# doughtmw/hmd-ego-pose

Hardware: AMD Instinct MI355X
Metric: frames/sec at 256x256 bs16 EfficientPose-phi0; ADD(-S) vs ref (higher is better)
Workload: dtype bf16; 1 GPU; EfficientPose phi=0 256x256 bf16 batch=16 per GPU: forward (stem, MBConv, BiFPN, 5 heads) + box/translation decode; seeded random-init weights, N(0,1) frames resident in HBM; 4 batches of 16 in flight per GPU on 4 HIP streams; phi=0, size=256, batch_per_gpu=16, global_batch=16, parallelism=dp1, batches_in_flight=4, anchors=12276, submission_threads=4

## Files before the change

### hmd_ego_pose_amd/csrc/hep_api.cpp

```cpp
#include <stdio.h>
#include <stdlib.h>
#include <string.h>

#include <math.h>

#include <chrono>
#include <fstream>
#include <memory>

#include "hep.h"
#include "hep_api_util.h"
#include "hep_plan.h"

using namespace hep;

thread_local std::string hep::g_err;

struct hep_handle { Session s; };

namespace hep {

Session::~Session() {
  if (!realised) return;
  for (auto& g : graphs) for (hipGraphExec_t ge : g.second) hipGraphExecDestroy(ge);
// ... 1070 lines not shown
  return calibrate_fp8(s, frames_nchw_device, batch);
} HEP_CATCH_INT

static std::string kernel_symbol(const Session& s, const Op& o) {
  const char* t = s.dtype ? "true" : "false";
  const int prec = o.kind == OP_PW ? (o.pw.fp8 ? 2 : (s.dtype ? 1 : 0)) : 0;
  char tmp[128];
  switch (o.kind) {
    case OP_STEM: if (o.stem.mfma) snprintf(tmp, sizeof tmp, "stem_kernel<%s, %d>", t, (o.stem.Cout + 15) / 16);
                  else snprintf(tmp, sizeof tmp, "stem_valu_kernel<%s>", t);
                  break;
    case OP_PW: { const int sev = pw_se_variant(o.pw);
                  const bool w8 = o.pw.nwv == 8 && prec == 0 && o.pw.mode == 2 && o.pw.act != ACT_SWISH && (sev == 0 || sev == 3) && o.pw.NT <= 2;
                  const bool fr = o.pw.frag && prec != 2 && o.pw.MT == 2 && o.pw.NT <= PW_FRAG_MAX_NT && o.pw.mode == 2 && sev >= 1 && o.pw.act != ACT_SWISH;
                  snprintf(tmp, sizeof tmp, fr ? "pw_gemm_kernel<%d, %d, %d, %d, %d, %d, %d, true>" : "pw_gemm_kernel<%d, %d, %d, %d, %d, %d, %d>", prec, o.pw.MT, o.pw.NT, o.pw.mode, o.pw.act == ACT_SWISH ? 1 : 0, sev, (w8 || (fr && o.pw.nwv == 8 && prec == 0 && sev == 3 && o.pw.NT <= 2)) ? 8 : 4); break; }
    case OP_DW: snprintf(tmp, sizeof tmp, "dw_kernel<%s, %d, %d, %d>", t, o.dw.k, o.dw.s, o.dw.TW); break;
    case OP_POOL: snprintf(tmp, sizeof tmp, "pool_kernel<%s>", t); break;
    case OP_PWG: snprintf(tmp, sizeof tmp, "pw_group_kernel<%s>", t); break;
    case OP_CHAIN: if (const int id = chain_shape_id(o.chain)) snprintf(tmp, sizeof tmp, "chain_shape_kernel<true, %d>", id);
                   else snprintf(tmp, sizeof tmp, "chain_kernel<%s, %d>", o.chain.bf16 ? "true" : "false", o.chain.stream_w);
                   break;
    case OP_SE: snprintf(tmp, sizeof tmp, "se_finish_kernel<%s>", t); break;
    case OP_MBF: { const int mp = o.mbf.has_expand && o.mbf.npass > 1 ? (o.mbf.mp_resident ? 2 : 1) : 0;
                   if (const int id = mbf_shape_id(o.mbf)) snprintf(tmp, sizeof tmp, "mbf_shape_kernel<%s, %d, %d, %d, %d, %d>", t, o.mbf.k, o.mbf.s, o.mbf.ts, mp, id);
                   else snprintf(tmp, sizeof tmp, "mbf_kernel<%s, %d, %d, %d, %s, %d>", t, o.mbf.k, o.mbf.s, o.mbf.ts, o.mbf.fp8 ? "true" : "false", mp);
                   break; }
#ifdef HEP_ALT
    case OP_SBF: snprintf(tmp, sizeof tmp, "sbf_kernel<%s>", t); break;
    case OP_LATE: snprintf(tmp, sizeof tmp, "late_kernel"); break;
    case OP_HEADS: snprintf(tmp, sizeof tmp, "heads_kernel"); break;
#endif
    case OP_XBF: { const int sp = xbf_specialised(o.xbf);
                   if (const int id = xbf_shape_id(o.xbf)) snprintf(tmp, sizeof tmp, "xbf_kernel_shape<true, %d>", id);
                   else snprintf(tmp, sizeof tmp, "xbf_kernel<%s, %d, %d, %d, %d, %d, %d, %d>", t, o.xbf.k, o.xbf.s, o.xbf.toh, o.xbf.tow, o.xbf.NT1, sp ? o.xbf.K1 : 0, sp ? o.xbf.NT2 : 0); break; }
    default: if (o.sep.direct) snprintf(tmp, sizeof tmp, "%s<%s, %d, %s>", o.sep.coop ? "tower_coop_kernel" : "tower_kernel", t, o.sep.C, o.sep.direct == 2 ? "true" : "false");
             else {
               const int mode = o.sep.chain ? 2 : (o.sep.nseg == 1 ? 0 : 1);
               const bool wl = o.sep.bf16 && o.sep.off_wpw && mode != 1;
               if (const int id = mode == 0 ? sep_shape_id(o.sep) : 0) snprintf(tmp, sizeof tmp, "sep_shape_kernel<true, %d>", id);
               else if (mode == 0 && sep_w8(o.sep)) snprintf(tmp, sizeof tmp, "sep_kernel<%s, 0, false, true>", t);
               else snprintf(tmp, sizeof tmp, wl ? "sep_kernel<%s, %d, true, false>" : "sep_kernel<%s, %d, false, false>", t, mode);
             }
             break;
  }
  return tmp;
}

// ... 124 lines not shown
```

### hmd_ego_pose_amd/csrc/hep_internal.h

```cpp
#pragma once
#include <hip/hip_runtime.h>
#include <stdint.h>

struct hep_sync;
struct GDSyncFailed { int rc; };

static constexpr inline uint32_t rcp_u32(uint32_t d) { return d <= 1 ? 0u : (uint32_t)(0x100000000ull / d) + 1u; }

#define HEP_MAX_SRC 3
#define SEP_MAX_TILES_N 6
#define SEP_MAX_TILES_MAP 24

enum { ACT_NONE = 0, ACT_SWISH = 1, ACT_SIGMOID = 2 };
enum { SRC_SAME = 1, SRC_UP = 2, SRC_DOWN = 3 };

struct StemArgs {
  const float* in; int64_t sn, sc, sh, sw;
  const float* w;
  const float* bias;
  void* out;
  int B, H, W, Ho, Wo, Cout, pad_t, pad_l, bf16;
  int mpw; uint32_t tx_rcp, ho_rcp;
  int mfma;
};
// ... 529 lines not shown
int backbone_tensor_count(const BGPlan&);
void backbone_tensor_offsets(const BGPlan&, int64_t* offsets);
int backbone_stage_count(const BGPlan&);
int backbone_stage(const BGPlan&, int i, char name[32], int64_t dims[4], int64_t* offset_floats);
void launch_backbone_forward(const BGPlan&, const float* params, const float* image, const float* branch_scale, float* const taps[3], float* ws, hipStream_t,
                             float momentum = 0.0f, float* stats_out = nullptr, const hep_sync* sync = nullptr);
void launch_backbone_backward(const BGPlan&, const float* const grad_taps[3], const float* branch_scale, float* grad_params, float* grad_image, float* ws,
                              hipStream_t, const hep_sync* sync = nullptr);

void launch_stem(const StemArgs&, hipStream_t);
int stem_uses_mfma(int cout, int force = -1);
void launch_pw(const PwArgs&, hipStream_t);
int pw_se_variant(const PwArgs&);
void launch_pwg(const PwgArgs&, hipStream_t);
void launch_dw(const DwArgs&, hipStream_t);
void launch_pool(const PoolArgs&, hipStream_t);
void launch_mbf(const MbfArgs&, hipStream_t);
size_t mbf_lds_layout(int Cin, int CC, int k, int s, int bf16, int has_expand, int max_inside, int ts, MbfArgs* a, int kp = 0);
int mbf_mp_fits(int CC, int kp, int bf16, int max_inside, int ts);
int mbf_mp_resident(int Cin, int CC, int max_inside, int ts);
int mbf_max_inside(int H, int W, int k, int s, int pad_t, int pad_l, int ts);
int mbf_prepare(void);
int mbf_shape_id(const MbfArgs&);
void launch_sep(const SepArgs&, hipStream_t);
void launch_tower(const SepArgs&, hipStream_t);
#define TOWER_BIAS_MAX 384
#define TOWER_WLDS_MAX (56 * 1024)
constexpr int tower_hdr_tiles(int C, bool bf16, int cap = 6) {
  if (!bf16) return 12;
  const long es = bf16 ? 2 : 4, wp = C + (bf16 ? 8 : 4), kstep = bf16 ? 32 : 16, ks = (C + kstep - 1) / kstep;
  const long fixed = 9L * C * 4 + 4L * ks * 64 * 16;
  const long room = TOWER_WLDS_MAX < 158L * 1024 - fixed ? TOWER_WLDS_MAX : 158L * 1024 - fixed;
  const long t = room / (16 * wp * es + 64);
  return t < 1 ? 1 : (t > cap ? cap : (int)t);
}
constexpr int tower_coop_hdr_tiles(int C, bool bf16) { return bf16 && C == 64 ? 36 : tower_hdr_tiles(C, bf16, 12); }
int tower_prepare(void);
int tower_coop_supported(int C, int bf16);
int tower_supports(int C);
int tower_map_tiles(int C);
void launch_decode(const DecodeArgs&, hipStream_t);
void launch_export(const ExportArgs&, hipStream_t);
void launch_preprocess(const PreprocArgs&, hipStream_t);
void launch_filter(const FilterArgs&, hipStream_t);
int filter_prepare(void);
void launch_amax_bf16(const void* x, int64_t n, unsigned* out , hipStream_t);
// ... 6 lines not shown
```

### hmd_ego_pose_amd/csrc/hep_plan.cpp

```cpp
#include <stdio.h>
#include <string.h>

#include <algorithm>
#include <cmath>
#include <map>

#include "hep.h"
#include "hep_plan.h"

namespace hep {

static const float kFusionEps = 1e-4f;

static void mbf_hpart_slot(Op& o, int seg, int idx, void* p) { SLOT(mbf.hpart)(o, seg, idx, p); SLOT(mbf.tail.hpart)(o, seg, idx, p); }

struct Planner {
  Session* s; const Pack& pk; std::string* err; WBuilder wb; bool ok = true;
  std::vector<Ref>& refs;
  int& ntails;
  const Knobs kn;
  std::map<int, int> front_of_out, front_of_part;
  Planner(Session* s_, const Pack& p, Plan* plan, std::string* e) : s(s_), pk(p), err(e), refs(plan->refs), ntails(plan->ntails), kn(s_->knobs) { wb.dtype = s_->dtype; wb.layout_only = plan->layout_only; }

  int tensor(const std::string& name, int H, int W, int C, bool f32 = false) {
// ... 343 lines not shown
      if (!boundary) flush_project();
      if (!ok) return -1;
    }
    auto dw_op = [&](OpKind kind, const std::string& name) {
      snprintf(nm, sizeof nm, "b%d.se_hpart", i);
      part_t = tensor(nm, 1, nblk, sqp, true);
      return new_op(kind, name);
    };
    auto dw_refs = [&](int op, Slot w, Slot bias, Slot se_wr, Slot in, Slot out, Slot part) {
      wref(op, w, wb.put_f32(wdw)); wref(op, bias, wb.put_f32(bn1.shift)); wref(op, se_wr, wr_off);
      if (in) tref(op, in, x, false);
      tref(op, out, dw_t, true); tref(op, part, part_t, true);
      Op& o = s->ops[op];
      o.act_bytes_per_image = ((double)Hin * Win + (double)Ho * Wo) * b.cexp * es();
      o.weight_bytes = (double)b.k * b.k * b.cexp * 4;
      o.flops_per_image = 2.0 * b.k * b.k * Ho * Wo * b.cexp;
    };
    auto mbf_op = [&](const char* suffix, int cin, int cc, int ts_, int has_expand, int max_in_, int npass_, int kp_) {
      nblk = ((Ho + ts_ - 1) / ts_) * ((Wo + ts_ - 1) / ts_) * ((b.cexp + cc - 1) / cc);
      const int op = dw_op(OP_MBF, "b" + std::to_string(i) + suffix);
      MbfArgs& m = s->ops[op].mbf;
      m.H = Hin; m.W = Win; m.Cin = cin; m.Cexp = b.cexp; m.Ho = Ho; m.Wo = Wo; m.k = b.k; m.s = b.stride;
      m.pad_t = pt; m.pad_l = pl; m.has_expand = has_expand; m.bf16 = s->dtype; m.CC = cc; m.sq = b.se; m.sqp = sqp; m.ts = ts_;
      m.npass = npass_; m.kp = kp_; m.generic = kn.mbf_generic != 0;
      mbf_lds_layout(cin, cc, b.k, b.stride, s->dtype, has_expand, max_in_, ts_, &m, kp_);
      front_of_out[dw_t] = op; front_of_part[part_t] = op;
      return op;
    };
    if (boundary) {
    } else if (CC) {
      if (!b.expand) CC = std::min(CC, b.cexp);
      const int op = mbf_op(".front", b.cin, CC, ts, b.expand, max_in, npass, kp);
      MbfArgs& m = s->ops[op].mbf;
      m.mp_resident = npass > 1 && mbf_mp_resident(b.cin, CC, max_in, ts) && kn.mbf_mp_res != 0;
      if (b.expand) {
        const PackTensor* w = get(p + "._expand_conv.conv.weight", {b.cexp, b.cin, 1, 1});
        BnFold bn0; if (!fold_bn(pk, p + "._bn0", b.cexp, &bn0, err)) ok = false;
        if (!ok) return -1;
        const int rows = (b.cexp + 15) / 16 * 16;
        const FoldedPw f = fold_pw(w, b.cin, nullptr, &bn0, 0, b.cexp, rows);
        if (s->dtype == 2) {
          std::vector<float> sc;
          wref(op, SLOT(mbf.we), wb.put_fp8(f.w, rows, b.cin, (b.cin + 15) & ~15, &sc)); wref(op, SLOT(mbf.we_scale), wb.put_f32(sc));
          m.fp8 = 1; m.a_scale = 1.f;
        } else wref(op, SLOT(mbf.we), wb.put_typed(f.w));
        wref(op, SLOT(mbf.be), wb.put_f32(bn0.shift));
      }
// ... 811 lines not shown
```

### hmd_ego_pose_amd/csrc/k_mbf.hip

```cpp
#include <stddef.h>
#include <stdio.h>
#include <stdlib.h>

#include <algorithm>

#include <type_traits>

#include "k_mbf_impl.h"

int mbf_shape_prepare_16(void); int mbf_shape_prepare_8(void);
bool launch_mbf_shape_16(int id, const MbfArgs&, dim3 grid, hipStream_t);
bool launch_mbf_shape_8(int id, const MbfArgs&, dim3 grid, hipStream_t);
void mbf_trace_bind_16(unsigned long long*); void mbf_trace_bind_8(unsigned long long*);

#ifdef HEP_MBF_TRACE
extern "C" int hep_dbg_mbf_trace(unsigned long long* host, int max_waves, int enable) {
  static unsigned long long* buf = nullptr;
  const size_t cap = (size_t)1 << 21;
  if (!buf) { if (hipMalloc((void**)&buf, cap * 8) != hipSuccess) return -1; hipMemset(buf, 0, cap * 8); }
  unsigned long long* p = enable ? buf : nullptr;
  mbf_trace_bind_tu(p); mbf_trace_bind_16(p); mbf_trace_bind_8(p);
  if (host) { hipDeviceSynchronize(); hipMemcpy(host, buf, (size_t)max_waves * 64, hipMemcpyDeviceToHost); }
  return (int)(cap / 8);
}
// ... 44 lines not shown
int mbf_mp_resident(int Cin, int CC, int max_inside, int ts) {
  const long items = (long)(((CC + 15) / 16) * 16 + max_inside) * (Cin / 8);
  return Cin % 8 == 0 && items <= 6L * mbf_threads(ts);
}

template <bool BF16, int KS, int S, int TS>
static int prep_one() {
  int rc = hipFuncSetAttribute(reinterpret_cast<const void*>(mbf_kernel<BF16, KS, S, TS, false, 0>), hipFuncAttributeMaxDynamicSharedMemorySize, 159 * 1024) == hipSuccess ? 0 : -1;
  rc |= hipFuncSetAttribute(reinterpret_cast<const void*>(mbf_kernel<BF16, KS, S, TS, false, 1>), hipFuncAttributeMaxDynamicSharedMemorySize, 159 * 1024) == hipSuccess ? 0 : -1;
  rc |= hipFuncSetAttribute(reinterpret_cast<const void*>(mbf_kernel<BF16, KS, S, TS, false, 2>), hipFuncAttributeMaxDynamicSharedMemorySize, 159 * 1024) == hipSuccess ? 0 : -1;
#ifdef HEP_WITH_FP8
  if constexpr (BF16) rc |= hipFuncSetAttribute(reinterpret_cast<const void*>(mbf_kernel<true, KS, S, TS, true, 0>), hipFuncAttributeMaxDynamicSharedMemorySize, 159 * 1024) == hipSuccess ? 0 : -1;
#endif
  return rc;
}
int mbf_prepare(void) {
  return prep_one<true, 3, 1, 8>() | prep_one<true, 3, 2, 8>() | prep_one<true, 5, 1, 8>() | prep_one<true, 5, 2, 8>() |
         prep_one<false, 3, 1, 8>() | prep_one<false, 3, 2, 8>() | prep_one<false, 5, 1, 8>() | prep_one<false, 5, 2, 8>() |
         prep_one<true, 3, 1, 16>() | prep_one<true, 5, 1, 16>() | prep_one<false, 3, 1, 16>() | prep_one<false, 5, 1, 16>() |
         mbf_shape_prepare_16() | mbf_shape_prepare_8();
}

int mbf_shape_id(const MbfArgs& a) {
  if (a.generic || a.fp8 || a.se_tail) return 0;
  const int mp = a.has_expand && a.npass > 1 ? (a.mp_resident ? 2 : 1) : 0;
#define X(id, bf, ks, s_, ts_, mp_, cin, cexp, cc, h, w, ho, wo, pt, pl, sq_, sqp_, he, of) \
  if ((a.bf16 != 0) == bf && a.k == ks && a.s == s_ && a.ts == ts_ && mp == mp_ && a.Cin == cin && a.Cexp == cexp && a.CC == cc && a.H == h && a.W == w && \
      a.Ho == ho && a.Wo == wo && a.pad_t == pt && a.pad_l == pl && a.sq == sq_ && a.sqp == sqp_ && (a.has_expand != 0) == (he != 0) && (a.out_frag != 0) == (of != 0)) return id;
  MBF_SHAPES(X)
#undef X
  return 0;
}

template <bool BF16, bool F8, int MP>
static void launch_mbf_t(const MbfArgs& a, dim3 grid, hipStream_t s) {
  if (a.ts == 16) {
    if (a.k == 3) hipLaunchKernelGGL((mbf_kernel<BF16, 3, 1, 16, F8, MP>), grid, dim3(1024), a.lds_bytes, s, a);
    else hipLaunchKernelGGL((mbf_kernel<BF16, 5, 1, 16, F8, MP>), grid, dim3(1024), a.lds_bytes, s, a);
  }
  else if (a.k == 3 && a.s == 1) hipLaunchKernelGGL((mbf_kernel<BF16, 3, 1, 8, F8, MP>), grid, dim3(512), a.lds_bytes, s, a);
  else if (a.k == 3 && a.s == 2) hipLaunchKernelGGL((mbf_kernel<BF16, 3, 2, 8, F8, MP>), grid, dim3(512), a.lds_bytes, s, a);
  else if (a.k == 5 && a.s == 1) hipLaunchKernelGGL((mbf_kernel<BF16, 5, 1, 8, F8, MP>), grid, dim3(512), a.lds_bytes, s, a);
  else hipLaunchKernelGGL((mbf_kernel<BF16, 5, 2, 8, F8, MP>), grid, dim3(512), a.lds_bytes, s, a);
}
void launch_mbf(const MbfArgs& a_, hipStream_t s) {
  MbfArgs a = a_;
#ifdef HEP_MBF_TRACE
  {
    static const char* sel = getenv("HEP_MBF_TRACE_SEL");
    int c = 0, h = 0;
    if (sel) sscanf(sel, "%d,%d", &c, &h);
    a.trace = !sel || (a.Cexp == c && a.H == h);
  }
#endif
  const int tiles = ((a.Wo + a.ts - 1) / a.ts) * ((a.Ho + a.ts - 1) / a.ts), chunks = (a.Cexp + a.CC - 1) / a.CC;
  dim3 grid(tiles * chunks, a.B);
  a.chunks = chunks; a.tiles_x = (a.Wo + a.ts - 1) / a.ts;
  a.chunks_rcp = rcp_u32(chunks); a.tiles_x_rcp = rcp_u32(a.tiles_x); a.gx_rcp = rcp_u32(grid.x);
#ifdef HEP_WITH_FP8
  if (a.bf16 && a.fp8) { launch_mbf_t<true, true, 0>(a, grid, s); return; }
#endif
  const int mp = a.has_expand && a.npass > 1 ? (a.mp_resident ? 2 : 1) : 0;
  a.vk_rcp = rcp_u32((uint32_t)std::max(1, a.Cin >> 3)); a.kpv_rcp = rcp_u32((uint32_t)std::max(1, a.kp >> 3));
  if (const int id = mbf_shape_id(a)) {
    if (launch_mbf_shape_16(id, a, grid, s) || launch_mbf_shape_8(id, a, grid, s)) return;
  }
  if (a.bf16) { if (mp == 2) launch_mbf_t<true, false, 2>(a, grid, s); else if (mp == 1) launch_mbf_t<true, false, 1>(a, grid, s); else launch_mbf_t<true, false, 0>(a, grid, s); }
  else { if (mp == 2) launch_mbf_t<false, false, 2>(a, grid, s); else if (mp == 1) launch_mbf_t<false, false, 1>(a, grid, s); else launch_mbf_t<false, false, 0>(a, grid, s); }
}
```

### hmd_ego_pose_amd/csrc/k_mbf_impl.h

```cpp
#pragma once
#include "hep_dev.h"
#include "hep_internal.h"
#include "se_finish.h"

#define MBF_SHAPES_16(X) \
  X(1, true, 5, 1, 16, 0,   40,  240, 64, 32, 32, 32, 32, 2, 2, 10, 16, 1, 0) \
  X(3, true, 3, 1, 16, 0,   80,  480, 64, 16, 16, 16, 16, 1, 1, 20, 24, 1, 1) \
  X(4, true, 5, 1, 16, 0,   80,  480, 64, 16, 16, 16, 16, 2, 2, 20, 24, 1, 1) \
  X(5, true, 5, 1, 16, 0,  112,  672, 64, 16, 16, 16, 16, 2, 2, 28, 32, 1, 1)
#define MBF_SHAPES_8(X) \
  X(2, true, 3, 2,  8, 0,   40,  240, 64, 32, 32, 16, 16, 0, 0, 10, 16, 1, 1) \
  X(6, true, 5, 2,  8, 0,  112,  672, 64, 16, 16,  8,  8, 1, 1, 28, 32, 1, 1) \
  X(7, true, 5, 1,  8, 0,  192, 1152, 64,  8,  8,  8,  8, 2, 2, 48, 48, 1, 1) \
  X(8, true, 3, 1,  8, 0,  192, 1152, 64,  8,  8,  8,  8, 1, 1, 48, 48, 1, 1)
#define MBF_SHAPES(X) MBF_SHAPES_16(X) MBF_SHAPES_8(X)

struct MbfShape { int Cin, Cexp, CC, H, W, Ho, Wo, pad_t, pad_l, sq, sqp, has_expand, out_frag; };
constexpr MbfShape mbf_shape(int d) {
  switch (d) {
#define X(id, bf, ks, s, ts, mp, cin, cexp, cc, h, w, ho, wo, pt, pl, sq, sqp, he, of) case id: return MbfShape{cin, cexp, cc, h, w, ho, wo, pt, pl, sq, sqp, he, of};
    MBF_SHAPES(X)
#undef X
    default: return MbfShape{};
  }
}


#ifdef HEP_MBF_TRACE
static __device__ unsigned long long* g_mbf_trace = nullptr;
static inline void mbf_trace_bind_tu(unsigned long long* p) { hipMemcpyToSymbol(HIP_SYMBOL(g_mbf_trace), &p, sizeof p); }
#ifdef HEP_MBF_TRACE_A
#define MSTAMP(i) do { if ((i) == 0 || (i) == 6) stamps[i] = __builtin_amdgcn_s_memrealtime(); } while (0)
#define XSTAMP(i) do { stamps[i] = __builtin_amdgcn_s_memrealtime(); } while (0)
#else
#define MSTAMP(i) do { stamps[i] = __builtin_amdgcn_s_memrealtime(); } while (0)
#define XSTAMP(i)
#endif
#else
#define MSTAMP(i)
#define XSTAMP(i)
#endif


template <bool BF16, int KS, int S, int TS, bool F8, int MP, int D>
__device__ __forceinline__ void mbf_body(const MbfArgs& a) {
  constexpr int MBF_THREADS = TS == 16 ? 1024 : 512, MBF_WAVES = MBF_THREADS / 64;
  constexpr MbfShape SH = mbf_shape(D);
  const int Cexp = D ? SH.Cexp : a.Cexp, CC = D ? SH.CC : a.CC, H = D ? SH.H : a.H, W = D ? SH.W : a.W, Ho = D ? SH.Ho : a.Ho, Wo = D ? SH.Wo : a.Wo;
  const int pad_t = D ? SH.pad_t : a.pad_t, pad_l = D ? SH.pad_l : a.pad_l, sq = D ? SH.sq : a.sq, sqp = D ? SH.sqp : a.sqp;
  const int has_expand = D ? SH.has_expand : a.has_expand, out_frag = D ? SH.out_frag : a.out_frag;
  [[maybe_unused]] const int se_tail = D ? 0 : a.se_tail;
  constexpr int TX_C = (SH.Wo + TS - 1) / TS, CH_C = SH.CC ? (SH.Cexp + SH.CC - 1) / SH.CC : 0, GX_C = TX_C * ((SH.Ho + TS - 1) / TS) * CH_C;
  const int tiles_x = D ? TX_C : a.tiles_x;
  const unsigned ngx = D ? (unsigned)GX_C : gridDim.x;
  const uint32_t chunks_rcp = D ? rcp_u32(CH_C) : a.chunks_rcp, tiles_x_rcp = D ? rcp_u32(TX_C) : a.tiles_x_rcp, gx_rcp = D ? rcp_u32(GX_C) : a.gx_rcp;
  typedef Vec8<BF16> V;
  typedef typename V::elem T;
  typedef Frag<BF16> F;
  typedef typename F::raw raw_t;
  constexpr int KSTEP = F::KSTEP, KLANE = F::KLANE, PAD = BF16 ? 8 : 4;
  constexpr int PW = (TS - 1) * S + KS;
  constexpr int PIN = PW * PW;
  extern __shared__ __attribute__((aligned(16))) unsigned char smem[];
  HEP_POISON(smem, a.lds_bytes);
#ifdef HEP_MBF_TRACE
  unsigned long long stamps[8] = {0, 0, 0, 0, 0, 0, 0, 0};
  MSTAMP(0);
#endif
  const int lane = threadIdx.x & 63, wave = __builtin_amdgcn_readfirstlane(threadIdx.x >> 6);
  const int r = lane & 15, g = lane >> 4;
  const int chunks = D ? CH_C : a.chunks;
  const int logical = xcd_remap(blockIdx.x + blockIdx.y * ngx, ngx * gridDim.y);
  const int b = udiv_rcp(logical, gx_rcp), bxl = logical - b * (int)ngx;
  const int tile = udiv_rcp(bxl, chunks_rcp), chunk = bxl - tile * chunks;
  const int tile_y = udiv_rcp(tile, tiles_x_rcp);
  const int oy0 = tile_y * TS, ox0 = (tile - tile_y * tiles_x) * TS;
  const int iy0 = oy0 * S - pad_t, ix0 = ox0 * S - pad_l;
  const int c0 = chunk * CC;
  const int cc = min(CC, Cexp - c0);
  const int K = D ? SH.Cin : a.Cin;
  const int KP = (MP ? a.kp : K) + PAD, EP = CC + PAD;
  T* a_s = reinterpret_cast<T*>(smem);
  T* e_s = reinterpret_cast<T*>(smem + a.off_e);
  T* w_s = reinterpret_cast<T*>(smem + a.off_we);
  float* wdw_s = reinterpret_cast<float*>(smem + a.off_w);
  float* be_s = wdw_s + KS * KS * CC;
  float* bdw_s = be_s + CC;
  const int K16 = (K + 15) & ~15, KP8 = K16 + 16;
  unsigned char* w8_s = smem + a.off_we;

  const int ntiles = (cc + 15) / 16;
  const int ksteps = (K + KSTEP - 1) / KSTEP;
  const int r0 = max(0, -iy0), r1 = min(PW, H - iy0), q0 = max(0, -ix0), q1 = min(PW, W - ix0);
  const int wi = q1 - q0, n_in = wi * (r1 - r0);
  const float wi_inv = __builtin_amdgcn_rcpf((float)wi);
  auto row_of = [&](int m) { return (int)(((float)m + 0.5f) * wi_inv); };
  constexpr int NDW = (KS * KS * 128 / 4 + MBF_THREADS - 1) / MBF_THREADS;
  const int cv = cc >> 2;
  const int cvsh = cv <= 2 ? 1 : 32 - __builtin_clz(cv - 1);
  f32x4 wv[NDW];
#ifdef HEP_MBF_TRACE_A
  asm volatile("s_waitcnt lgkmcnt(0)" ::: "memory");
#endif
  XSTAMP(1);
  const float* wdw_g = a.wdw + c0;
#pragma unroll
  for (int j = 0; j < NDW; j++) {
    const int i = threadIdx.x + j * MBF_THREADS, tap = i >> cvsh, c4 = i & ((1 << cvsh) - 1);
    const bool ok = tap < KS * KS && c4 < cv;
    wv[j] = *reinterpret_cast<const f32x4*>(wdw_g + (ok ? (uint32_t)(tap * Cexp + c4 * 4) : 0u));
  }
  const int bi = threadIdx.x;
  const bool b_dw = bi < cv, b_ex = has_expand && bi >= 64 && bi - 64 < cv;
  const f32x4 bv = *reinterpret_cast<const f32x4*>((b_ex ? a.be : a.bdw) + c0 + (b_dw || b_ex ? (uint32_t)(bi & 63) * 4 : 0u));
  auto park_weights = [&]() {
#pragma unroll
    for (int j = 0; j < NDW; j++) {
      const int i = threadIdx.x + j * MBF_THREADS, tap = i >> cvsh, c4 = i & ((1 << cvsh) - 1);
      if (tap < KS * KS && c4 < cv) *reinterpret_cast<f32x4*>(wdw_s + tap * CC + c4 * 4) = wv[j];
    }
    if (b_dw) *reinterpret_cast<f32x4*>(bdw_s + bi * 4) = bv;
    else if (b_ex) *reinterpret_cast<f32x4*>(be_s + (bi - 64) * 4) = bv;
  };
  {
    constexpr int NB = BF16 ? 8 : 4;
    constexpr int VB = 8 * (int)sizeof(T);
    const int vecs = has_expand ? K >> 3 : cc >> 3;
// ... 169 lines not shown
            d[0] = w0[j]; if (!BF16) d[1] = w1[j];
          }
        }
      };
      auto issue_p = [&](int base) {
#pragma unroll
        for (int j = 0; j < NH; j++) {
          const int mm = base + j * rstride + row0, m = min(mm, n_in - 1), ri = row_of(m);
          const uint32_t off = (uint32_t)((pix0 + ri * W + (m - ri * wi)) * K) * (uint32_t)sizeof(T) + (uint32_t)(v * VB);
          const unsigned char* src = in_b + (vok && mm < n_in ? off : 0u);
          p0[j] = *reinterpret_cast<const raw_t*>(src); if (!BF16) p1[j] = *reinterpret_cast<const raw_t*>(src + 16);
        }
      };
      auto store_p = [&](int base) {
#pragma unroll
        for (int j = 0; j < NH; j++) {
          const int m = base + j * rstride + row0;
          if (vok && m < n_in) {
            raw_t* d = reinterpret_cast<raw_t*>(a_s + m * KP + v * 8);
            d[0] = p0[j]; if (!BF16) d[1] = p1[j];
          }
        }
      };
      issue_w(0); issue_p(0);
      XSTAMP(2); park_weights(); XSTAMP(3);
      store_w(0); store_p(0);
      for (int base = rstride * NH; base < n_wrows; base += rstride * NH) { issue_w(base); store_w(base); }
      for (int base = rstride * NH; base < n_in; base += rstride * NH) { issue_p(base); store_p(base); }
    } else {
      for (int base = 0; base < PIN; base += rstride * NB) {
        raw_t x0[NB], x1[NB];
        bool inside[NB];
#pragma unroll
        for (int j = 0; j < NB; j++) {
          const int p = base + j * rstride + row0, ty = p / PW, gy = iy0 + ty, gx = ix0 + p - ty * PW;
          inside[j] = p < PIN && v < vecs && gy >= 0 && gy < H && gx >= 0 && gx < W;
          const uint32_t off = (uint32_t)((gy * W + gx) * K + c0) * (uint32_t)sizeof(T) + (uint32_t)(v * VB);
          const unsigned char* src = in_b + (inside[j] ? off : 0u);
          x0[j] = *reinterpret_cast<const raw_t*>(src); if (!BF16) x1[j] = *reinterpret_cast<const raw_t*>(src + 16);
        }
        if (base == 0) { XSTAMP(2); park_weights(); XSTAMP(3); }
#pragma unroll
        for (int j = 0; j < NB; j++) {
          const int p = base + j * rstride + row0;
          if (p < PIN && v < vecs) {
            raw_t* d = reinterpret_cast<raw_t*>(e_s + p * EP + v * 8);
            d[0] = inside[j] ? x0[j] : raw_t{}; if (!BF16) d[1] = inside[j] ? x1[j] : raw_t{};
          }
        }
      }
    }
  }
  if constexpr (MP == 0) {
  MSTAMP(1); XSTAMP(4);
  __syncthreads();
  MSTAMP(2); XSTAMP(5);
  }

  if (MP == 0 && has_expand) {
    const int mpairs = (n_in + 31) >> 5;
    const int ntsh = ntiles <= 1 ? 0 : 32 - __builtin_clz(ntiles - 1);
    constexpr int KSMAX = BF16 ? 6 : 12;
    if (!F8 && ksteps <= KSMAX && (1 << ntsh) <= MBF_WAVES) {
      const int nt = wave & ((1 << ntsh) - 1), grp = wave >> ntsh, ngrp = MBF_WAVES >> ntsh;
      const int n = nt * 16 + 4 * g;
      if (nt < ntiles) {
        raw_t wfr[KSMAX];
        const T* wrow = w_s + (nt * 16 + r) * KP;
#pragma unroll
        for (int ks = 0; ks < KSMAX; ks++) {
          const bool kok = ks < ksteps && ks * KSTEP + KLANE * g < K;
          wfr[ks] = *reinterpret_cast<const raw_t*>(wrow + (kok ? ks * KSTEP + KLANE * g : 0));
          if (!kok) wfr[ks] = raw_t{};
        }
        const f32x4 bias = *reinterpret_cast<const f32x4*>(be_s + min(n, cc - 4));
        const int mtiles = (n_in + 15) >> 4;
        for (int mt = grp; mt < mtiles; mt += 2 * ngrp) {
          const int m0 = mt * 16 + r, m1 = m0 + 16 * ngrp;
          const T* arow0 = a_s + min(m0, n_in - 1) * KP;
          const T* arow1 = a_s + min(m1, n_in - 1) * KP;
          f32x4 acc0 = bias, acc1 = bias;
// ... 66 lines not shown
          if (m < n_in) {
            const f32x4 acc = half ? acc1 : acc0;
            const int ri = row_of(m), p = (r0 + ri) * PW + q0 + (m - ri * wi);
            float v[4];
#pragma unroll
            for (int q = 0; q < 4; q++) v[q] = F8 ? fmaf(acc[q], ws[q], bias[q]) : acc[q] + bias[q];
            swish_n<BF16, 4>(v);
            V::store4(e_s, (int64_t)p * EP + n, v);
          }
        }
      }
    }
    MSTAMP(3);
    __syncthreads();
  }
  if constexpr (MP == 0) { MSTAMP(4); }

  const int cqs = cc >> 2;
  const int cqsh = cqs <= 1 ? 0 : 32 - __builtin_clz(cqs - 1), cqp = 1 << cqsh;
  constexpr bool SPLIT = TS == 8;
  constexpr int HALF = SPLIT ? MBF_THREADS / 2 : MBF_THREADS;
  const int half = SPLIT ? threadIdx.x / HALF : 0, tl = SPLIT ? threadIdx.x % HALF : threadIdx.x;
  const int cq = tl & (cqp - 1), qd = tl >> cqsh;
  f32x4* xch = reinterpret_cast<f32x4*>(smem);
  float sum[4] = {0, 0, 0, 0};
  const bool item = cq < cqs && qd < TS * TS / 4;
  constexpr int KH = SPLIT ? (KS + 1) / 2 : KS;
  constexpr int NX = 3 * S + KS;
  const int py = qd / (TS / 4), px = (qd % (TS / 4)) * 4;
  float acc[4][4];
  if (item) {
    {
      const f32x4 b0 = *reinterpret_cast<const f32x4*>(bdw_s + cq * 4);
#pragma unroll
      for (int j = 0; j < 4; j++)
#pragma unroll
        for (int c = 0; c < 4; c++) acc[j][c] = half ? 0.f : b0[c];
    }
#pragma unroll 1
    for (int ky = half ? KH : 0; ky < (half ? KS : KH); ky++) {
      f32x4 wr[KS];
#pragma unroll
      for (int kx = 0; kx < KS; kx++) wr[kx] = *reinterpret_cast<const f32x4*>(wdw_s + (ky * KS + kx) * CC + cq * 4);
      const int64_t erow = (int64_t)((py * S + ky) * PW + px * S) * EP + cq * 4;
#pragma unroll
      for (int hx = 0; hx < NX; hx++) {
        float ev[4];
// ... 34 lines not shown
    };
    if (oy < Ho) {
      float sp[2][4] = {{0.f, 0.f, 0.f, 0.f}, {0.f, 0.f, 0.f, 0.f}};
#pragma unroll
      for (int j = 0; j < 4; j++) {
        if (ox + j < Wo) {
          float v[4];
#pragma unroll
          for (int c = 0; c < 4; c++) v[c] = acc[j][c];
          swish_n<BF16, 4>(v);
#pragma unroll
          for (int c = 0; c < 4; c++) sp[j >> 1][c] += v[c];
          ostore(ox + j, v);
        }
      }
#pragma unroll
      for (int c = 0; c < 4; c++) sum[c] = sp[0][c] + sp[1][c];
    }
  }
  MSTAMP(5);

  if (a.hpart) {
    constexpr int NWC = HALF / 64;
    float* ssum = reinterpret_cast<float*>(smem + a.off_e);
    const int part = threadIdx.x & 7, ch = part * 8;
    const int jp = threadIdx.x >> 3;
    f32x4 wp0, wp1;
    {
      const f32x4* wp = reinterpret_cast<const f32x4*>(a.se_wr + (int64_t)min(jp, sq - 1) * Cexp + c0 + min(ch, max(cc - 8, 0)));
      wp0 = wp[0]; wp1 = wp[1];
    }
    if (wave < NWC) {
      for (int off = cqp; off < 64; off <<= 1) {
#pragma unroll
        for (int c = 0; c < 4; c++) sum[c] += __shfl_xor(sum[c], off, 64);
      }
      if (lane < cqs) *reinterpret_cast<f32x4*>(ssum + wave * CC + lane * 4) = (f32x4){sum[0], sum[1], sum[2], sum[3]};
    }
    __syncthreads();
    float cs[8] = {0, 0, 0, 0, 0, 0, 0, 0};
    if (ch < cc) {
#pragma unroll
      for (int w4 = 0; w4 < NWC; w4++) {
        const f32x4* sp = reinterpret_cast<const f32x4*>(ssum + w4 * CC + ch);
        const f32x4 s0 = sp[0], s1 = sp[1];
#pragma unroll
        for (int c = 0; c < 4; c++) { cs[c] += s0[c]; cs[4 + c] += s1[c]; }
// ... 29 lines not shown
        const bool last = __hip_atomic_fetch_add(cnt, 1u, __ATOMIC_RELAXED, __HIP_MEMORY_SCOPE_AGENT) + 1u == ngx;
        if (last) __hip_atomic_store(cnt, 0u, __ATOMIC_RELAXED, __HIP_MEMORY_SCOPE_AGENT);
        *flag = last;
      }
      __syncthreads();
      if (*flag) se_finish_body<BF16, MBF_THREADS, true>(a.tail, b, 0, a.tail.C, threadIdx.x, reinterpret_cast<float*>(smem) + 32);
    }
#endif
  }
#ifdef HEP_MBF_TRACE
  MSTAMP(6);
  if (g_mbf_trace && a.trace && lane == 0) {
    unsigned long long* o = g_mbf_trace + ((size_t)(b * ngx + bxl) * MBF_WAVES + wave) * 8;
    for (int i = 0; i < 7; i++) o[i] = stamps[i];
    o[7] = __builtin_amdgcn_s_getreg((4 << 0) | (0 << 6) | (31 << 11));
  }
#endif
}

template <bool BF16, int KS, int S, int TS, bool F8, int MP>
__global__ __launch_bounds__(TS == 16 ? 1024 : 512) void mbf_kernel(MbfArgs a) { mbf_body<BF16, KS, S, TS, F8, MP, 0>(a); }
template <bool BF16, int KS, int S, int TS, int MP, int D>
__global__ __launch_bounds__(TS == 16 ? 1024 : 512) void mbf_shape_kernel(MbfArgs a) { mbf_body<BF16, KS, S, TS, false, MP, D>(a); }

#define MBF_SHAPE_TU(ROWS, PREPARE, LAUNCH, BIND) \
  int PREPARE(void) { \
    int rc = 0; \
    ROWS(MBF_SHAPE_PREP_ROW) \
    return rc; \
  } \
  bool LAUNCH(int id, const MbfArgs& a, dim3 grid, hipStream_t s) { \
    switch (id) { \
      ROWS(MBF_SHAPE_LAUNCH_ROW) \
      default: return false; \
    } \
  } \
  void BIND(unsigned long long* p) { MBF_TRACE_BIND_TU(p); }
#define MBF_SHAPE_PREP_ROW(id, bf, ks, s_, ts, mp, ...) \
  rc |= hipFuncSetAttribute(reinterpret_cast<const void*>(mbf_shape_kernel<bf, ks, s_, ts, mp, id>), hipFuncAttributeMaxDynamicSharedMemorySize, 159 * 1024) == hipSuccess ? 0 : -1;
#define MBF_SHAPE_LAUNCH_ROW(id, bf, ks, s_, ts, mp, ...) \
  case id: hipLaunchKernelGGL((mbf_shape_kernel<bf, ks, s_, ts, mp, id>), grid, dim3(ts == 16 ? 1024 : 512), a.lds_bytes, s, a); return true;
#ifdef HEP_MBF_TRACE
#define MBF_TRACE_BIND_TU(p) mbf_trace_bind_tu(p)
#else
#define MBF_TRACE_BIND_TU(p) (void)(p)
#endif
```

Baseline: 61350 frames/s.

## Feed MBConv expand GEMM A-operand directly from global into registers for whole-map shapes

For three specialised MBConv shapes where one tile covers the whole feature map, the expand 1x1 GEMM now loads input fragments straight from global memory into registers. This skips staging the input patch in LDS, and the kernel keeps two n-tiles of weight fragments in registers. A smaller compile-time LDS layout is used, and the exchange buffer is moved to the weight region. The old staged path stays available as a separate kernel via a knob value of 2. The aim is to cut LDS traffic and staging synchronisation, at the cost of more register pressure and uncoalesced per-lane global loads.

```diff
diff --git a/hmd_ego_pose_amd/csrc/hep_api.cpp b/hmd_ego_pose_amd/csrc/hep_api.cpp
--- a/hmd_ego_pose_amd/csrc/hep_api.cpp
+++ b/hmd_ego_pose_amd/csrc/hep_api.cpp
@@ -1116,7 +1116,7 @@
                    break;
     case OP_SE: snprintf(tmp, sizeof tmp, "se_finish_kernel<%s>", t); break;
     case OP_MBF: { const int mp = o.mbf.has_expand && o.mbf.npass > 1 ? (o.mbf.mp_resident ? 2 : 1) : 0;
-                   if (const int id = mbf_shape_id(o.mbf)) snprintf(tmp, sizeof tmp, "mbf_shape_kernel<%s, %d, %d, %d, %d, %d>", t, o.mbf.k, o.mbf.s, o.mbf.ts, mp, id);
+                   if (const int id = mbf_shape_id(o.mbf)) snprintf(tmp, sizeof tmp, "%s<%s, %d, %d, %d, %d, %d>", o.mbf.generic == 2 && mbf_shape_direct(id) ? "mbf_shape_staged_kernel" : "mbf_shape_kernel", t, o.mbf.k, o.mbf.s, o.mbf.ts, mp, id);
                    else snprintf(tmp, sizeof tmp, "mbf_kernel<%s, %d, %d, %d, %s, %d>", t, o.mbf.k, o.mbf.s, o.mbf.ts, o.mbf.fp8 ? "true" : "false", mp);
                    break; }
 #ifdef HEP_ALT
diff --git a/hmd_ego_pose_amd/csrc/hep_internal.h b/hmd_ego_pose_amd/csrc/hep_internal.h
--- a/hmd_ego_pose_amd/csrc/hep_internal.h
+++ b/hmd_ego_pose_amd/csrc/hep_internal.h
@@ -575,6 +575,7 @@
 int mbf_max_inside(int H, int W, int k, int s, int pad_t, int pad_l, int ts);
 int mbf_prepare(void);
 int mbf_shape_id(const MbfArgs&);
+int mbf_shape_direct(int id);
 void launch_sep(const SepArgs&, hipStream_t);
 void launch_tower(const SepArgs&, hipStream_t);
 #define TOWER_BIAS_MAX 384
diff --git a/hmd_ego_pose_amd/csrc/hep_plan.cpp b/hmd_ego_pose_amd/csrc/hep_plan.cpp
--- a/hmd_ego_pose_amd/csrc/hep_plan.cpp
+++ b/hmd_ego_pose_amd/csrc/hep_plan.cpp
@@ -389,7 +389,7 @@
       MbfArgs& m = s->ops[op].mbf;
       m.H = Hin; m.W = Win; m.Cin = cin; m.Cexp = b.cexp; m.Ho = Ho; m.Wo = Wo; m.k = b.k; m.s = b.stride;
       m.pad_t = pt; m.pad_l = pl; m.has_expand = has_expand; m.bf16 = s->dtype; m.CC = cc; m.sq = b.se; m.sqp = sqp; m.ts = ts_;
-      m.npass = npass_; m.kp = kp_; m.generic = kn.mbf_generic != 0;
+      m.npass = npass_; m.kp = kp_; m.generic = kn.mbf_generic == 2 ? 2 : (kn.mbf_generic != 0);
       mbf_lds_layout(cin, cc, b.k, b.stride, s->dtype, has_expand, max_in_, ts_, &m, kp_);
       front_of_out[dw_t] = op; front_of_part[part_t] = op;
       return op;
diff --git a/hmd_ego_pose_amd/csrc/k_mbf.hip b/hmd_ego_pose_amd/csrc/k_mbf.hip
--- a/hmd_ego_pose_amd/csrc/k_mbf.hip
+++ b/hmd_ego_pose_amd/csrc/k_mbf.hip
@@ -90,15 +90,17 @@
 }
 
 int mbf_shape_id(const MbfArgs& a) {
-  if (a.generic || a.fp8 || a.se_tail) return 0;
+  if (a.generic == 1 || a.fp8 || a.se_tail) return 0;
   const int mp = a.has_expand && a.npass > 1 ? (a.mp_resident ? 2 : 1) : 0;
-#define X(id, bf, ks, s_, ts_, mp_, cin, cexp, cc, h, w, ho, wo, pt, pl, sq_, sqp_, he, of) \
+#define X(id, bf, ks, s_, ts_, mp_, cin, cexp, cc, h, w, ho, wo, pt, pl, sq_, sqp_, he, of, ad) \
   if ((a.bf16 != 0) == bf && a.k == ks && a.s == s_ && a.ts == ts_ && mp == mp_ && a.Cin == cin && a.Cexp == cexp && a.CC == cc && a.H == h && a.W == w && \
-      a.Ho == ho && a.Wo == wo && a.pad_t == pt && a.pad_l == pl && a.sq == sq_ && a.sqp == sqp_ && (a.has_expand != 0) == (he != 0) && (a.out_frag != 0) == (of != 0)) return id;
+      a.Ho == ho && a.Wo == wo && a.pad_t == pt && a.pad_l == pl && a.sq == sq_ && a.sqp == sqp_ && (a.has_expand != 0) == (he != 0) && (a.out_frag != 0) == (of != 0) && \
+      (!ad || mbf_direct_lds(id).lds_bytes <= a.lds_bytes)) return id;
   MBF_SHAPES(X)
 #undef X
   return 0;
 }
+int mbf_shape_direct(int id) { return mbf_shape(id).a_direct; }
 
 template <bool BF16, bool F8, int MP>
 static void launch_mbf_t(const MbfArgs& a, dim3 grid, hipStream_t s) {
@@ -131,6 +133,10 @@
   const int mp = a.has_expand && a.npass > 1 ? (a.mp_resident ? 2 : 1) : 0;
   a.vk_rcp = rcp_u32((uint32_t)std::max(1, a.Cin >> 3)); a.kpv_rcp = rcp_u32((uint32_t)std::max(1, a.kp >> 3));
   if (const int id = mbf_shape_id(a)) {
+    if (mbf_shape_direct(id) && a.generic != 2) {
+      const MbfLds l = mbf_direct_lds(id);
+      a.off_e = l.off_e; a.off_we = l.off_we; a.off_w = l.off_w; a.lds_bytes = l.lds_bytes;
+    }
     if (launch_mbf_shape_16(id, a, grid, s) || launch_mbf_shape_8(id, a, grid, s)) return;
   }
   if (a.bf16) { if (mp == 2) launch_mbf_t<true, false, 2>(a, grid, s); else if (mp == 1) launch_mbf_t<true, false, 1>(a, grid, s); else launch_mbf_t<true, false, 0>(a, grid, s); }
diff --git a/hmd_ego_pose_amd/csrc/k_mbf_impl.h b/hmd_ego_pose_amd/csrc/k_mbf_impl.h
--- a/hmd_ego_pose_amd/csrc/k_mbf_impl.h
+++ b/hmd_ego_pose_amd/csrc/k_mbf_impl.h
@@ -4,24 +4,42 @@
 #include "se_finish.h"
 
 #define MBF_SHAPES_16(X) \
-  X(1, true, 5, 1, 16, 0,   40,  240, 64, 32, 32, 32, 32, 2, 2, 10, 16, 1, 0) \
-  X(3, true, 3, 1, 16, 0,   80,  480, 64, 16, 16, 16, 16, 1, 1, 20, 24, 1, 1) \
-  X(4, true, 5, 1, 16, 0,   80,  480, 64, 16, 16, 16, 16, 2, 2, 20, 24, 1, 1) \
-  X(5, true, 5, 1, 16, 0,  112,  672, 64, 16, 16, 16, 16, 2, 2, 28, 32, 1, 1)
+  X(1, true, 5, 1, 16, 0,   40,  240, 64, 32, 32, 32, 32, 2, 2, 10, 16, 1, 0, 0) \
+  X(3, true, 3, 1, 16, 0,   80,  480, 64, 16, 16, 16, 16, 1, 1, 20, 24, 1, 1, 1) \
+  X(4, true, 5, 1, 16, 0,   80,  480, 64, 16, 16, 16, 16, 2, 2, 20, 24, 1, 1, 1) \
+  X(5, true, 5, 1, 16, 0,  112,  672, 64, 16, 16, 16, 16, 2, 2, 28, 32, 1, 1, 0)
 #define MBF_SHAPES_8(X) \
-  X(2, true, 3, 2,  8, 0,   40,  240, 64, 32, 32, 16, 16, 0, 0, 10, 16, 1, 1) \
-  X(6, true, 5, 2,  8, 0,  112,  672, 64, 16, 16,  8,  8, 1, 1, 28, 32, 1, 1) \
-  X(7, true, 5, 1,  8, 0,  192, 1152, 64,  8,  8,  8,  8, 2, 2, 48, 48, 1, 1) \
-  X(8, true, 3, 1,  8, 0,  192, 1152, 64,  8,  8,  8,  8, 1, 1, 48, 48, 1, 1)
+  X(2, true, 3, 2,  8, 0,   40,  240, 64, 32, 32, 16, 16, 0, 0, 10, 16, 1, 1, 0) \
+  X(6, true, 5, 2,  8, 0,  112,  672, 64, 16, 16,  8,  8, 1, 1, 28, 32, 1, 1, 1) \
+  X(7, true, 5, 1,  8, 0,  192, 1152, 64,  8,  8,  8,  8, 2, 2, 48, 48, 1, 1, 0) \
+  X(8, true, 3, 1,  8, 0,  192, 1152, 64,  8,  8,  8,  8, 1, 1, 48, 48, 1, 1, 0)
 #define MBF_SHAPES(X) MBF_SHAPES_16(X) MBF_SHAPES_8(X)
 
-struct MbfShape { int Cin, Cexp, CC, H, W, Ho, Wo, pad_t, pad_l, sq, sqp, has_expand, out_frag; };
+struct MbfShape { int Cin, Cexp, CC, H, W, Ho, Wo, pad_t, pad_l, sq, sqp, has_expand, out_frag, a_direct; };
 constexpr MbfShape mbf_shape(int d) {
   switch (d) {
-#define X(id, bf, ks, s, ts, mp, cin, cexp, cc, h, w, ho, wo, pt, pl, sq, sqp, he, of) case id: return MbfShape{cin, cexp, cc, h, w, ho, wo, pt, pl, sq, sqp, he, of};
+#define X(id, bf, ks, s, ts, mp, cin, cexp, cc, h, w, ho, wo, pt, pl, sq, sqp, he, of, ad) case id: return MbfShape{cin, cexp, cc, h, w, ho, wo, pt, pl, sq, sqp, he, of, ad};
     MBF_SHAPES(X)
 #undef X
     default: return MbfShape{};
+  }
+}
+
+struct MbfLds { size_t off_e, off_we, off_w, lds_bytes; };
+constexpr size_t mbf_up16(size_t v) { return (v + 15) & ~(size_t)15; }
+constexpr size_t mbf_max_sz(size_t x, size_t y) { return x > y ? x : y; }
+constexpr MbfLds mbf_direct_lds_of(int k, int s, int ts, int Cin, int CC) {
+  const size_t pw = (size_t)(ts - 1) * s + k, pin = pw * pw;
+  const size_t e_bytes = mbf_up16(mbf_max_sz(pin * (CC + 8) * 2, (size_t)16 * CC * 4));
+  const size_t we_bytes = mbf_up16(mbf_max_sz((size_t)CC * (Cin + 8) * 2, ts == 8 ? (size_t)4 * 256 * 16 : 0));
+  return MbfLds{0, e_bytes, e_bytes + we_bytes, e_bytes + we_bytes + (size_t)(k * k + 2) * CC * 4};
+}
+constexpr MbfLds mbf_direct_lds(int d) {
+  switch (d) {
+#define X(id, bf, ks, s, ts, mp, cin, cexp, cc, h, w, ho, wo, pt, pl, sq, sqp, he, of, ad) case id: return ad ? mbf_direct_lds_of(ks, s, ts, cin, cc) : MbfLds{};
+    MBF_SHAPES(X)
+#undef X
+    default: return MbfLds{};
   }
 }
 
@@ -42,10 +60,15 @@
 #endif
 
 
-template <bool BF16, int KS, int S, int TS, bool F8, int MP, int D>
+template <bool BF16, int KS, int S, int TS, bool F8, int MP, int D, bool STG = false>
 __device__ __forceinline__ void mbf_body(const MbfArgs& a) {
   constexpr int MBF_THREADS = TS == 16 ? 1024 : 512, MBF_WAVES = MBF_THREADS / 64;
   constexpr MbfShape SH = mbf_shape(D);
+  constexpr bool DIRECT = D > 0 && SH.a_direct != 0 && !STG;
+  constexpr MbfLds LD = mbf_direct_lds(D);
+  static_assert(!DIRECT || (BF16 && !F8 && MP == 0 && SH.has_expand && SH.Ho <= TS && SH.Wo <= TS && (TS - 1) * S + KS - SH.pad_t >= SH.H && (TS - 1) * S + KS - SH.pad_l >= SH.W &&
+                            (SH.H * SH.W) % 16 == 0 && SH.CC % 32 == 0 && SH.Cexp % 32 == 0 && SH.Cin % 8 == 0), "direct rows: one tile = the whole map, whole pairs of n-tiles");
+  const size_t off_e = DIRECT ? LD.off_e : a.off_e, off_we = DIRECT ? LD.off_we : a.off_we, off_w = DIRECT ? LD.off_w : a.off_w;
   const int Cexp = D ? SH.Cexp : a.Cexp, CC = D ? SH.CC : a.CC, H = D ? SH.H : a.H, W = D ? SH.W : a.W, Ho = D ? SH.Ho : a.Ho, Wo = D ? SH.Wo : a.Wo;
   const int pad_t = D ? SH.pad_t : a.pad_t, pad_l = D ? SH.pad_l : a.pad_l, sq = D ? SH.sq : a.sq, sqp = D ? SH.sqp : a.sqp;
   const int has_expand = D ? SH.has_expand : a.has_expand, out_frag = D ? SH.out_frag : a.out_frag;
@@ -80,10 +103,10 @@
   const int cc = min(CC, Cexp - c0);
   const int K = D ? SH.Cin : a.Cin;
   const int KP = (MP ? a.kp : K) + PAD, EP = CC + PAD;
-  T* a_s = reinterpret_cast<T*>(smem);
-  T* e_s = reinterpret_cast<T*>(smem + a.off_e);
-  T* w_s = reinterpret_cast<T*>(smem + a.off_we);
-  float* wdw_s = reinterpret_cast<float*>(smem + a.off_w);
+  [[maybe_unused]] T* a_s = reinterpret_cast<T*>(smem);
+  T* e_s = reinterpret_cast<T*>(smem + off_e);
+  T* w_s = reinterpret_cast<T*>(smem + off_we);
+  float* wdw_s = reinterpret_cast<float*>(smem + off_w);
   float* be_s = wdw_s + KS * KS * CC;
   float* bdw_s = be_s + CC;
   const int K16 = (K + 15) & ~15, KP8 = K16 + 16;
@@ -103,6 +126,21 @@
   asm volatile("s_waitcnt lgkmcnt(0)" ::: "memory");
 #endif
   XSTAMP(1);
+  constexpr int HW_D = SH.H * SH.W, MT_D = HW_D / 16, MPW = DIRECT ? MT_D / MBF_WAVES : 1, KS_D = DIRECT ? (SH.Cin + KSTEP - 1) / KSTEP : 1;
+  static_assert(!DIRECT || (MPW >= 1 && MPW * MBF_WAVES == MT_D && KS_D <= 4), "direct rows: whole m-tiles per wave, two n-tiles of weight fragments in registers");
+  [[maybe_unused]] raw_t xa_d[MPW * KS_D];
+  if constexpr (DIRECT) {
+    const unsigned char* in_d = reinterpret_cast<const unsigned char*>(a.in) + (int64_t)b * HW_D * SH.Cin * (int)sizeof(T);
+#pragma unroll
+    for (int i = 0; i < MPW; i++) {
+      const int m = min((wave + i * MBF_WAVES) * 16 + r, HW_D - 1);
+#pragma unroll
+      for (int ks = 0; ks < KS_D; ks++) {
+        const int k = ks * KSTEP + KLANE * g;
+        xa_d[i * KS_D + ks] = *reinterpret_cast<const raw_t*>(in_d + (uint32_t)(m * SH.Cin + (k < SH.Cin ? k : 0)) * (uint32_t)sizeof(T));
+      }
+    }
+  }
   const float* wdw_g = a.wdw + c0;
 #pragma unroll
   for (int j = 0; j < NDW; j++) {
@@ -318,10 +356,11 @@
           }
         }
       };
-      issue_w(0); issue_p(0);
+      issue_w(0); if constexpr (!DIRECT) issue_p(0);
       XSTAMP(2); park_weights(); XSTAMP(3);
-      store_w(0); store_p(0);
+      store_w(0); if constexpr (!DIRECT) store_p(0);
       for (int base = rstride * NH; base < n_wrows; base += rstride * NH) { issue_w(base); store_w(base); }
+      if constexpr (!DIRECT)
       for (int base = rstride * NH; base < n_in; base += rstride * NH) { issue_p(base); store_p(base); }
     } else {
       for (int base = 0; base < PIN; base += rstride * NB) {
@@ -353,6 +392,52 @@
   MSTAMP(2); XSTAMP(5);
   }
 
+  if constexpr (DIRECT) {
+    constexpr int NTB = 2;
+#pragma unroll
+    for (int nt = 0; nt < SH.CC / 16; nt += NTB) {
+      if (nt < ntiles) {
+        raw_t wf[NTB][KS_D];
+        const T* wrow = w_s + (nt * 16 + r) * KP;
+#pragma unroll
+        for (int ks = 0; ks < KS_D; ks++) {
+          const bool kok = ks * KSTEP + KLANE * g < K;
+          const int ko = kok ? ks * KSTEP + KLANE * g : 0;
+#pragma unroll
+          for (int h = 0; h < NTB; h++) {
+            wf[h][ks] = *reinterpret_cast<const raw_t*>(wrow + h * 16 * KP + ko);
+            if (!kok) wf[h][ks] = raw_t{};
+          }
+        }
+        const int n = nt * 16 + 4 * g;
+        f32x4 bias[NTB];
+#pragma unroll
+        for (int h = 0; h < NTB; h++) bias[h] = *reinterpret_cast<const f32x4*>(be_s + n + 16 * h);
+#pragma unroll
+        for (int i = 0; i < MPW; i++) {
+          f32x4 acc[NTB];
+#pragma unroll
+          for (int h = 0; h < NTB; h++) acc[h] = bias[h];
+#pragma unroll
+          for (int ks = 0; ks < KS_D; ks++)
+#pragma unroll
+            for (int h = 0; h < NTB; h++) acc[h] = F::mma(wf[h][ks], xa_d[i * KS_D + ks], acc[h]);
+          const int m = (wave + i * MBF_WAVES) * 16 + r;
+          const int ri = row_of(m), p = (r0 + ri) * PW + q0 + (m - ri * wi);
+#pragma unroll
+          for (int h = 0; h < NTB; h++) {
+            float v[4];
+#pragma unroll
+            for (int q = 0; q < 4; q++) v[q] = acc[h][q];
+            swish_n<BF16, 4>(v);
+            V::store4(e_s, (int64_t)p * EP + n + 16 * h, v);
+          }
+        }
+      }
+    }
+    MSTAMP(3);
+    __syncthreads();
+  } else
   if (MP == 0 && has_expand) {
     const int mpairs = (n_in + 31) >> 5;
     const int ntsh = ntiles <= 1 ? 0 : 32 - __builtin_clz(ntiles - 1);
@@ -465,7 +550,7 @@
   constexpr int HALF = SPLIT ? MBF_THREADS / 2 : MBF_THREADS;
   const int half = SPLIT ? threadIdx.x / HALF : 0, tl = SPLIT ? threadIdx.x % HALF : threadIdx.x;
   const int cq = tl & (cqp - 1), qd = tl >> cqsh;
-  f32x4* xch = reinterpret_cast<f32x4*>(smem);
+  f32x4* xch = reinterpret_cast<f32x4*>(smem + (DIRECT ? off_we : 0));
   float sum[4] = {0, 0, 0, 0};
   const bool item = cq < cqs && qd < TS * TS / 4;
   constexpr int KH = SPLIT ? (KS + 1) / 2 : KS;
@@ -546,7 +631,7 @@
 
   if (a.hpart) {
     constexpr int NWC = HALF / 64;
-    float* ssum = reinterpret_cast<float*>(smem + a.off_e);
+    float* ssum = reinterpret_cast<float*>(smem + off_e);
     const int part = threadIdx.x & 7, ch = part * 8;
     const int jp = threadIdx.x >> 3;
     f32x4 wp0, wp1;
@@ -622,6 +707,23 @@
 __global__ __launch_bounds__(TS == 16 ? 1024 : 512) void mbf_kernel(MbfArgs a) { mbf_body<BF16, KS, S, TS, F8, MP, 0>(a); }
 template <bool BF16, int KS, int S, int TS, int MP, int D>
 __global__ __launch_bounds__(TS == 16 ? 1024 : 512) void mbf_shape_kernel(MbfArgs a) { mbf_body<BF16, KS, S, TS, false, MP, D>(a); }
+template <bool BF16, int KS, int S, int TS, int MP, int D>
+__global__ __launch_bounds__(TS == 16 ? 1024 : 512) void mbf_shape_staged_kernel(MbfArgs a) { mbf_body<BF16, KS, S, TS, false, MP, D, true>(a); }
+
+template <bool BF16, int KS, int S, int TS, int MP, int D>
+static int mbf_shape_prep_row() {
+  int rc = hipFuncSetAttribute(reinterpret_cast<const void*>(mbf_shape_kernel<BF16, KS, S, TS, MP, D>), hipFuncAttributeMaxDynamicSharedMemorySize, 159 * 1024) == hipSuccess ? 0 : -1;
+  if constexpr (mbf_shape(D).a_direct != 0)
+    rc |= hipFuncSetAttribute(reinterpret_cast<const void*>(mbf_shape_staged_kernel<BF16, KS, S, TS, MP, D>), hipFuncAttributeMaxDynamicSharedMemorySize, 159 * 1024) == hipSuccess ? 0 : -1;
+  return rc;
+}
+template <bool BF16, int KS, int S, int TS, int MP, int D>
+static void mbf_shape_launch_row(const MbfArgs& a, dim3 grid, hipStream_t s) {
+  if constexpr (mbf_shape(D).a_direct != 0) {
+    if (a.generic == 2) { hipLaunchKernelGGL((mbf_shape_staged_kernel<BF16, KS, S, TS, MP, D>), grid, dim3(TS == 16 ? 1024 : 512), a.lds_bytes, s, a); return; }
+  }
+  hipLaunchKernelGGL((mbf_shape_kernel<BF16, KS, S, TS, MP, D>), grid, dim3(TS == 16 ? 1024 : 512), a.lds_bytes, s, a);
+}
 
 #define MBF_SHAPE_TU(ROWS, PREPARE, LAUNCH, BIND) \
   int PREPARE(void) { \
@@ -637,9 +739,9 @@
   } \
   void BIND(unsigned long long* p) { MBF_TRACE_BIND_TU(p); }
 #define MBF_SHAPE_PREP_ROW(id, bf, ks, s_, ts, mp, ...) \
-  rc |= hipFuncSetAttribute(reinterpret_cast<const void*>(mbf_shape_kernel<bf, ks, s_, ts, mp, id>), hipFuncAttributeMaxDynamicSharedMemorySize, 159 * 1024) == hipSuccess ? 0 : -1;
+  rc |= mbf_shape_prep_row<bf, ks, s_, ts, mp, id>();
 #define MBF_SHAPE_LAUNCH_ROW(id, bf, ks, s_, ts, mp, ...) \
-  case id: hipLaunchKernelGGL((mbf_shape_kernel<bf, ks, s_, ts, mp, id>), grid, dim3(ts == 16 ? 1024 : 512), a.lds_bytes, s, a); return true;
+  case id: mbf_shape_launch_row<bf, ks, s_, ts, mp, id>(a, grid, s); return true;
 #ifdef HEP_MBF_TRACE
 #define MBF_TRACE_BIND_TU(p) mbf_trace_bind_tu(p)
 #else
```

After: 61800 frames/s, median of 6. About the same (+0.7%).
